# hellovuong/ORB_SLAM3_FAST

Measured on AMD Instinct MI355X. Metric: ORB extract+match frames/sec @1280×720 stereo (both-eye ORBextractor + ComputeStereoMatches), higher is better.
Workload: dtype u8; 1 GPU; C3: synthetic 1280x720 rectified stereo pairs, 1500 features, 8 levels, scale 1.2, FAST 20/7, ComputeStereoMatches (bf=0.12*532.03, b=0.12); handles=4, distinct_streams_per_gpu=32, frames_in_ring=3, stereo_matches_pair0=987, parallelism=independent stereo pairs sharded across GPUs, no data-path collective

## Files before the change

orb_slam3_fast_amd/csrc/orbx_kernels.hip:

```cpp
#include <type_traits>
#include <map>
#include <mutex>

#include "orbx_device.h"
#include "orbx_introsort.h"
#include "orbx_sincos.h"
#include "orbx_blur_mfma.h"

namespace orbx {

__constant__ int c_umax[16] = {15, 15, 15, 15, 14, 14, 14, 13, 13, 12, 11, 10, 9, 8, 6, 3};

#define RS_DW 256
#define RS_DR 16
#define RS_HROWS 6
struct ResizeLv {
  struct { int w, h, pitch, xcoef, ycoef; } D;
  struct { int w, h; } S;
  int sp, l;
  int nbx;
  const uint8_t* src; long long srcImg;
  uint8_t* dst; long long dstImg;
  const uint32_t* tiles;
  const uint32_t* rows;
// ... 683 lines not shown
  o.cpos = take(maxn * 8);
  o.e[0] = take(maxn * 8);
  o.e[1] = take(maxn * 8);
  o.mark = take(maxn * 2);
  o.bestk = take(maxn * 4);
  o.tsum = take(256 * 8 + 64);
  o.cellpre = take((maxcells + 1) * 4);
  o.total = off;
  return o;
}
__host__ __device__ inline int oct_maxn(const Geom& g, int l0, int l1) {
  int q = 0;
  for (int l = l0; l < l1; l++) q = g.lv[l].quota > q ? g.lv[l].quota : q;
  return q + 4 * kMaxIni + 8;
}
__host__ __device__ inline int oct_maxcells(const Geom& g, int l0, int l1) {
  int c = 0;
  for (int l = l0; l < l1; l++) c = g.lv[l].nCols * g.lv[l].nRows > c ? g.lv[l].nCols * g.lv[l].nRows : c;
  return c;
}
__host__ __device__ inline int oct_rep(const Geom& g, int l0, int l1) {
  const int maxn = oct_maxn(g, l0, l1), maxcells = oct_maxcells(g, l0, l1);
  if (oct_layout(maxn, maxcells, 2).total <= 78 * 1024) return 2;
  return 1;
}
size_t octree_lds_bytes(const Geom& g, int l0, int l1) {
  return (size_t)oct_layout(oct_maxn(g, l0, l1), oct_maxcells(g, l0, l1), oct_rep(g, l0, l1)).total;
}

__device__ __forceinline__ uint64_t wave0_scan_u64(uint64_t* v, int n) {
  const int lane = threadIdx.x;
  const uint64_t s = lane < n ? v[lane] : 0;
  const uint64_t incl = wave_scan_dpp_u64(s);
  if (lane < n) v[lane] = incl - s;
  return readlane_u64(incl, 63);
}
template <int NT>
__device__ __forceinline__ uint64_t block_scan_u64(uint64_t* v, int n, uint64_t* tsum) {
  const int tid = threadIdx.x, lane = tid & 63, wv = tid >> 6;
  const int per = (n + NT - 1) / NT;
  const int b = min(tid * per, n), e = min(b + per, n);
  uint64_t s = 0;
  for (int i = b; i < e; i++) s += v[i];
  const uint64_t incl = wave_scan_dpp_u64(s);
  if (lane == 63) tsum[wv] = incl;
  __syncthreads();
  uint64_t wbase = 0, total = 0;
#pragma unroll
  for (int w = 0; w < NT / 64; w++) {
    const uint64_t t = tsum[w];
    if (w < wv) wbase += t;
    total += t;
  }
  uint64_t run = wbase + incl - s;
  for (int i = b; i < e; i++) {
    const uint64_t t = v[i];
    v[i] = run;
    run += t;
  }
  __syncthreads();
  return total;
}

__device__ __forceinline__ int quadrant(int x, int y, int x0, int x1, int y0, int y1) {
  const int hx = (x1 - x0 + 1) >> 1, hy = (y1 - y0 + 1) >> 1;
  return (x < x0 + hx ? 0 : 1) | (y < y0 + hy ? 0 : 2);
}

constexpr int OCT_KMAX = 32;
constexpr int OCT_GROUP = 4;
template <bool REG, int NT>
struct OctCands {
  uint32_t rk[REG ? OCT_KMAX : 1];
  uint32_t rn2[REG ? OCT_KMAX / 2 : 1];
  uint32_t* keys;
  uint16_t* kn;
  int n;
  static constexpr uint32_t kNoCand = 0xFFFFu;
  template <class F>
  __device__ __forceinline__ void sweep(F f) {
    if constexpr (REG) {
#pragma unroll
      for (int j0 = 0; j0 < OCT_KMAX; j0 += OCT_GROUP) {
        if (j0 * NT >= n) continue;
#pragma unroll
        for (int j = j0; j < j0 + OCT_GROUP; j++)
        {
          uint32_t key = rk[j], nd = (rn2[j >> 1] >> (16 * (j & 1))) & 0xFFFFu;
          asm volatile("" : "+v"(key), "+v"(nd));
          if (nd != kNoCand) {
            f(0, key, nd);
            rn2[j >> 1] = (j & 1) ? (rn2[j >> 1] & 0xFFFFu) | (nd << 16) : (rn2[j >> 1] & 0xFFFF0000u) | nd;
          }
        }
        __builtin_amdgcn_sched_barrier(0);
      }
    } else {
      for (int k = threadIdx.x; k < n; k += NT) {
        uint32_t nd = kn[k];
        const uint32_t nd0 = nd;
        f(k, keys[k], nd);
        if (nd != nd0) kn[k] = (uint16_t)nd;
      }
    }
  }
  template <class F>
  __device__ __forceinline__ void fill(F f) {
    if constexpr (REG) {
#pragma unroll
      for (int j = 0; j < OCT_KMAX; j++) {
        const int k = (int)threadIdx.x + j * NT;
        rk[j] = 0;
        if (k < n) rk[j] = f(k);
      }
#pragma unroll
      for (int j = 0; j < OCT_KMAX; j++) {
        const int k = (int)threadIdx.x + j * NT;
        const uint32_t nd = k < n ? 0u : kNoCand;
        rn2[j >> 1] = (j & 1) ? rn2[j >> 1] | (nd << 16) : nd;
      }
    } else {
      for (int k = threadIdx.x; k < n; k += NT) {
        keys[k] = f(k);
        kn[k] = 0;
      }
    }
  }
};

struct OctCtx {
  int16_t *nx0, *nx1, *ny0, *ny1;
  uint32_t* ncnt;
  int nodeStride;
  uint32_t* cnt4;
  int nrep;
  uint32_t* cntr;
  uint16_t* cpos;
  uint64_t* scan;
  uint64_t* ebuf;
  uint16_t* mark;
  uint32_t* nmid;
  uint64_t* tsum;
  int* cellpre;
  int* s_i;
  int maxn;
  uint16_t* owner;
  int ownerBytes;
  uint8_t* tab;
  int tabBytes;
};

template <int NT, class CD>
__device__ __forceinline__ void octree_gather(CD& cd, const OctCtx& c, const LevelDev& L, int n, int cells,
                                              const uint32_t* __restrict__ sparse) {
  if (2 * n <= c.ownerBytes) {
    for (int cell = threadIdx.x; cell < cells; cell += NT) {
      const int b = c.cellpre[cell], e = min(c.cellpre[cell + 1], n);
      for (int i = b; i < e; i++) c.owner[i] = (uint16_t)cell;
    }
    __syncthreads();
    cd.fill([&](int k) {
      const int cell = c.owner[k];
      return sparse[(long long)cell * L.cellCap + (k - c.cellpre[cell])];
    });
    __syncthreads();
  } else {
    cd.fill([&](int k) {
      int lo = 0, hi = cells;
      while (hi - lo > 1) {
        const int mid = (lo + hi) >> 1;
        if (c.cellpre[mid] <= k) lo = mid; else hi = mid;
      }
      return sparse[(long long)lo * L.cellCap + (k - c.cellpre[lo])];
    });
  }
}

template <bool REG, int NT>
__device__ __forceinline__ void octree_body(const Geom& g, const LevelDev& L, const OctCtx& c, int n, int cells,
                                            const uint32_t* __restrict__ sparse, uint32_t* __restrict__ keys,
                                            uint16_t* __restrict__ kn, uint32_t* __restrict__ out,
                                            int* __restrict__ outCount, int profLevel) {
  const int tid = threadIdx.x;
#ifdef OCT_PROF
  long long tmk[96]; int nmk = 0;
#define MK() do { if (nmk < 96) tmk[nmk++] = wall_clock64(); } while (0)
#else
#define MK() do {} while (0)
#endif
  MK();
  OctCands<REG, NT> cd;
  cd.keys = keys;
  cd.kn = kn;
  cd.n = n;
  octree_gather<NT>(cd, c, L, n, cells, sparse);
  MK();
  const int N = L.quota;
  struct Buf {
    char* base;
    int stride;
    __device__ __forceinline__ int16_t* operator[](int b) const { return reinterpret_cast<int16_t*>(base + b * stride); }
  };
  struct BufU {
    char* base;
    int stride;
    __device__ __forceinline__ uint32_t* operator[](int b) const { return reinterpret_cast<uint32_t*>(base + b * stride); }
  };
  const Buf nx0{(char*)c.nx0, c.nodeStride}, nx1{(char*)c.nx1, c.nodeStride}, ny0{(char*)c.ny0, c.nodeStride},
      ny1{(char*)c.ny1, c.nodeStride};
  const BufU ncnt{(char*)c.ncnt, c.nodeStride};
  uint32_t* cnt4 = c.cnt4;
  uint32_t* cntr = c.cntr;
  const int nrep = c.nrep, rep = tid & (nrep - 1);
  auto zero_counters = [&](int nslots) {
    for (int i = tid; i < nslots * nrep; i += NT) cntr[i] = 0;
  };
  auto reduce_counters = [&](int nslots) {
    for (int i = tid; i < nslots; i += NT) {
      uint32_t v = 0;
      for (int r = 0; r < nrep; r++) v += cntr[i * nrep + r];
      cnt4[i] = v;
    }
  };
  uint16_t* cpos = c.cpos;
  uint64_t* scan = c.scan;
  uint16_t* mark = c.mark;
  uint32_t* nmid = c.nmid;
  uint64_t* tsum = c.tsum;
  auto pack_mid = [&](int b, int i) {
    const int x0 = nx0[b][i], x1 = nx1[b][i], y0 = ny0[b][i], y1 = ny1[b][i];
    return (uint32_t)(x0 + ((x1 - x0 + 1) >> 1)) | ((uint32_t)(y0 + ((y1 - y0 + 1) >> 1)) << 12) |
           (ncnt[b][i] > 1 ? 0x80000000u : 0u);
  };
  auto classify = [&](uint32_t key, uint32_t mid) {
    return (key_x(key) >= (int)(mid & 0xFFF) ? 1 : 0) | (key_y(key) >= (int)((mid >> 12) & 0xFFF) ? 2 : 0);
  };
  int* s_i = c.s_i;

  const int W = L.w - 2 * kBorder, H = L.h - 2 * kBorder;
  const int nIni = (int)roundf((float)W / (float)H);
  const float hX = (float)W / (float)nIni;

  zero_counters(kMaxIni);
  __syncthreads();
  cd.sweep([&](int, uint32_t key, uint32_t& nd) {
    const int r = (int)((float)key_x(key) / hX);
    nd = (uint32_t)r;
    atomicAdd(&cntr[r * nrep + rep], 1u);
  });
  __syncthreads();
  reduce_counters(kMaxIni);
  __syncthreads();
  if (tid == 0) {
    int na = 0;
    for (int i = 0; i < nIni; i++) {
      if (cnt4[i] == 0) {
        cpos[i] = 0xFFFF;
        continue;
      }
      nx0[0][na] = (int16_t)(int)(hX * (float)i);
      nx1[0][na] = (int16_t)(int)(hX * (float)(i + 1));
      ny0[0][na] = 0;
      ny1[0][na] = (int16_t)H;
      ncnt[0][na] = cnt4[i];
      cpos[i] = (uint16_t)na;
      na++;
    }
    s_i[0] = na;
    for (int i = 0; i < na; i++) nmid[i] = pack_mid(0, i);
  }
  __syncthreads();
  cd.sweep([&](int, uint32_t, uint32_t& nd) { nd = cpos[nd]; });
  int nA = s_i[0];
  int cur = 0;
  __syncthreads();

  MK();
  bool finish = false;
  int nE = 0, ecur = 0;
  while (!finish) {
    const int prevSize = nA;
    zero_counters(nA * 4);
    __syncthreads();
    MK();
    cd.sweep([&](int, uint32_t key, uint32_t& nd) {
      const uint32_t mid = nmid[nd];
      if (mid >> 31) {
        const int q = classify(key, mid);
        atomicAdd(&cntr[(nd * 4 + q) * nrep + rep], 1u);
        nd |= (uint32_t)q << 14;
      }
    });
    __syncthreads();
    reduce_counters(nA * 4);
    __syncthreads();
    MK();
    for (int i = tid; i < nA; i += NT) {
      uint64_t cc = 0, nm = 1, ce = 0;
      if (ncnt[cur][i] > 1) {
        nm = 0;
        for (int q = 0; q < 4; q++) {
          cc += cnt4[i * 4 + q] > 0;
          ce += cnt4[i * 4 + q] > 1;
        }
      }
      scan[i] = cc | (nm << 21) | (ce << 42);
    }
    __syncthreads();
    const uint64_t tot = block_scan_u64<NT>(scan, nA, tsum);
    MK();
    const int tc = (int)(tot & 0x1FFFFF), tnm = (int)((tot >> 21) & 0x1FFFFF), tce = (int)(tot >> 42);
    const int nxt = cur ^ 1;
    for (int i = tid; i < nA; i += NT) {
      const uint64_t pre = scan[i];
      const int pc = (int)(pre & 0x1FFFFF), pnm = (int)((pre >> 21) & 0x1FFFFF), pce = (int)(pre >> 42);
      if (ncnt[cur][i] > 1) {
        const int x0 = nx0[cur][i], x1 = nx1[cur][i], y0 = ny0[cur][i], y1 = ny1[cur][i];
        const int hx = (x1 - x0 + 1) >> 1, hy = (y1 - y0 + 1) >> 1;
        int cc = 0;
        for (int q = 0; q < 4; q++) cc += cnt4[i * 4 + q] > 0;
        const int base = tc - (pc + cc);
        int after = 0, eb = pce;
        for (int q = 0; q < 4; q++) {
          const uint32_t cq = cnt4[i * 4 + q];
          if (cq > 1) {
            int rank_after = 0;
            for (int q2 = q + 1; q2 < 4; q2++) rank_after += cnt4[i * 4 + q2] > 0;
            const int cx0 = (q & 1) ? x0 + hx : x0;
            (c.ebuf + ecur * c.maxn)[eb++] = ((uint64_t)cq << 28) | ((uint64_t)(uint32_t)cx0 << 16) | (uint64_t)(base + rank_after);
          }
        }
        for (int q = 3; q >= 0; q--) {
          const uint32_t cq = cnt4[i * 4 + q];
          if (cq == 0) continue;
          const int pos = base + after++;
          nx0[nxt][pos] = (int16_t)((q & 1) ? x0 + hx : x0);
          nx1[nxt][pos] = (int16_t)((q & 1) ? x1 : x0 + hx);
          ny0[nxt][pos] = (int16_t)((q & 2) ? y0 + hy : y0);
          ny1[nxt][pos] = (int16_t)((q & 2) ? y1 : y0 + hy);
          ncnt[nxt][pos] = cq;
          cpos[i * 4 + q] = (uint16_t)pos;
        }
      } else {
        const int pos = tc + pnm;
        nx0[nxt][pos] = nx0[cur][i];
        nx1[nxt][pos] = nx1[cur][i];
        ny0[nxt][pos] = ny0[cur][i];
        ny1[nxt][pos] = ny1[cur][i];
// ... 54 lines not shown
    __syncthreads();
    for (int m = tid; m < nE; m += NT) {
      const int nd = (int)(E[nE - 1 - m] & 0xFFFF);
      uint64_t cc = 0, ce = 0;
      for (int q = 0; q < 4; q++) {
        cc += cnt4[nd * 4 + q] > 0;
        ce += cnt4[nd * 4 + q] > 1;
      }
      scan[m] = cc | (ce << 21);
    }
    __syncthreads();
    block_scan_u64<NT>(scan, nE, tsum);
    for (int m = tid; m < nE; m += NT) {
      const int nd = (int)(E[nE - 1 - m] & 0xFFFF);
      int cc = 0;
      for (int q = 0; q < 4; q++) cc += cnt4[nd * 4 + q] > 0;
      const int cincl = (int)(scan[m] & 0x1FFFFF) + cc;
      if (nA + cincl - (m + 1) >= N) {
        atomicMin(&s_i[1], m + 1);
        s_i[2] = 1;
      }
    }
    __syncthreads();
    const int nP = s_i[1];
    const bool broke = s_i[2] != 0;
    int tc, tce;
    if (nP < nE) {
      tc = (int)(scan[nP] & 0x1FFFFF);
      tce = (int)(scan[nP] >> 21);
    } else {
      const int nd = (int)(E[0] & 0xFFFF);
      int cc = 0, ce = 0;
      for (int q = 0; q < 4; q++) {
        cc += cnt4[nd * 4 + q] > 0;
        ce += cnt4[nd * 4 + q] > 1;
      }
      tc = nE ? (int)(scan[nE - 1] & 0x1FFFFF) + cc : 0;
      tce = nE ? (int)(scan[nE - 1] >> 21) + ce : 0;
    }
    const int nxt = cur ^ 1;
    for (int m = tid; m < nP; m += NT) {
      const int nd = (int)(E[nE - 1 - m] & 0xFFFF);
      const int x0 = nx0[cur][nd], x1 = nx1[cur][nd], y0 = ny0[cur][nd], y1 = ny1[cur][nd];
      const int hx = (x1 - x0 + 1) >> 1, hy = (y1 - y0 + 1) >> 1;
      int cc = 0;
      for (int q = 0; q < 4; q++) cc += cnt4[nd * 4 + q] > 0;
      const int pc = (int)(scan[m] & 0x1FFFFF);
      int eb = (int)(scan[m] >> 21);
      const int base = tc - (pc + cc);
      for (int q = 0; q < 4; q++) {
        const uint32_t cq = cnt4[nd * 4 + q];
        if (cq > 1) {
          int rank_after = 0;
          for (int q2 = q + 1; q2 < 4; q2++) rank_after += cnt4[nd * 4 + q2] > 0;
          const int cx0 = (q & 1) ? x0 + hx : x0;
          E2[eb++] = ((uint64_t)cq << 28) | ((uint64_t)(uint32_t)cx0 << 16) | (uint64_t)(base + rank_after);
        }
      }
      int after = 0;
      for (int q = 3; q >= 0; q--) {
        const uint32_t cq = cnt4[nd * 4 + q];
        if (cq == 0) continue;
        const int pos = base + after++;
        nx0[nxt][pos] = (int16_t)((q & 1) ? x0 + hx : x0);
        nx1[nxt][pos] = (int16_t)((q & 1) ? x1 : x0 + hx);
        ny0[nxt][pos] = (int16_t)((q & 2) ? y0 + hy : y0);
        ny1[nxt][pos] = (int16_t)((q & 2) ? y1 : y0 + hy);
        ncnt[nxt][pos] = cq;
        cpos[nd * 4 + q] = (uint16_t)pos;
      }
    }
    __syncthreads();
    for (int i = tid; i < nA; i += NT) scan[i] = (mark[i] == 0 || mark[i] > nP) ? 1 : 0;
    __syncthreads();
    const int nKeep = (int)block_scan_u64<NT>(scan, nA, tsum);
    for (int i = tid; i < nA; i += NT) {
      if (mark[i] == 0 || mark[i] > nP) {
        const int pos = tc + (int)scan[i];
        nx0[nxt][pos] = nx0[cur][i];
        nx1[nxt][pos] = nx1[cur][i];
        ny0[nxt][pos] = ny0[cur][i];
        ny1[nxt][pos] = ny1[cur][i];
        ncnt[nxt][pos] = ncnt[cur][i];
        cpos[i * 4] = cpos[i * 4 + 1] = cpos[i * 4 + 2] = cpos[i * 4 + 3] = (uint16_t)pos;
      }
    }
    __syncthreads();
    cd.sweep([&](int, uint32_t, uint32_t& v) { v = cpos[(v & 0x3FFF) * 4 + (v >> 14)]; });
    for (int i = tid; i < tc + nKeep; i += NT) nmid[i] = pack_mid(nxt, i);
    __syncthreads();
    cur = nxt;
    nA = tc + nKeep;
    nE = tce;
    ecur ^= 1;
    MK();
    if (broke || nA == prevSize) finish = true;
  }

  MK();
  uint64_t* best = scan;
  uint64_t* bestr = reinterpret_cast<uint64_t*>(cntr);
  const int nrepB = nrep >= 2 ? nrep * 2 : 1, repB = tid & (nrepB - 1);
  if (nrepB > 1)
    for (int i = tid; i < nA * nrepB; i += NT) bestr[i] = 0;
  else
    for (int i = tid; i < nA; i += NT) best[i] = 0;
  __syncthreads();
  const float invH = 1.0f / (float)L.hCell, invW = 1.0f / (float)L.wCell;
  auto rank_key = [&](uint32_t key) {
    const int xr = key_x(key) - 3, yr = key_y(key) - 3;
    const int cy = (int)(((float)yr + 0.5f) * invH), cx = (int)(((float)xr + 0.5f) * invW);
    const uint32_t rank = (uint32_t)(((cy * L.nCols + cx) * L.hCell + (yr - cy * L.hCell)) * L.wCell + (xr - cx * L.wCell));
    return ((unsigned long long)key_r(key) << 32) | (0xFFFFFFFFu - rank);
  };
  if (nrepB > 1) {
    cd.sweep([&](int, uint32_t key, uint32_t& nd) {
      atomicMax((unsigned long long*)&bestr[nd * nrepB + repB], rank_key(key));
    });
    __syncthreads();
    for (int i = tid; i < nA; i += NT) {
      uint64_t v = 0;
      for (int r = 0; r < nrepB; r++) v = bestr[i * nrepB + r] > v ? bestr[i * nrepB + r] : v;
      best[i] = v;
    }
  } else {
    cd.sweep([&](int, uint32_t key, uint32_t& nd) { atomicMax((unsigned long long*)&best[nd], rank_key(key)); });
  }
  __syncthreads();
  const int nOut = min(nA, L.selCap);
  cd.sweep([&](int, uint32_t key, uint32_t& nd) {
    if ((int)nd < nOut && best[nd] == rank_key(key)) out[nd] = pack_key(key_x(key) + kBorder, key_y(key) + kBorder, key_r(key));
  });
  if (tid == 0) *outCount = nOut;
  MK();
#ifdef OCT_PROF
  if (tid == 0 && profLevel) {
    printf("n=%d nA=%d :", n, nA);
    for (int i = 1; i < nmk; i++) printf(" %d", (int)(tmk[i] - tmk[i - 1]));
    printf("\n");
  }
#endif
#undef MK
}

constexpr int OCT_HD = 5;
__host__ __device__ inline int oct_hbase(int nIni, int d) { return nIni * (((1 << (2 * d)) - 1) / 3); }
__host__ __device__ inline bool oct_hist_fits(int nIni) {
  return nIni <= 2 && oct_hbase(nIni, OCT_HD + 1) * 6 <= 16400 && nIni * (1 << (2 * OCT_HD)) * 2 <= 4096;
}

template <int NT>
__device__ __forceinline__ bool octree_hist_body(const Geom& g, const LevelDev& L, const OctCtx& c, int n, int cells,
                                                 const uint32_t* __restrict__ sparse, uint32_t* __restrict__ keys,
                                                 uint32_t* __restrict__ out, int* __restrict__ outCount, int prof) {
  const int tid = threadIdx.x;
#ifdef OCT_PROF
  long long hmk[48]; int nhmk = 0;
#define HMK() do { if (nhmk < 48) hmk[nhmk++] = wall_clock64(); } while (0)
#else
#define HMK() do {} while (0)
#endif
  HMK();
  OctCands<true, NT> cd;
  cd.keys = keys;
  cd.kn = nullptr;
  cd.n = n;
  octree_gather<NT>(cd, c, L, n, cells, sparse);
  HMK();
  const int N = L.quota;
  struct Buf {
    char* base;
    int stride;
    __device__ __forceinline__ int16_t* operator[](int b) const { return reinterpret_cast<int16_t*>(base + b * stride); }
  };
  struct BufU {
    char* base;
    int stride;
    __device__ __forceinline__ uint32_t* operator[](int b) const { return reinterpret_cast<uint32_t*>(base + b * stride); }
  };
  const Buf nx0{(char*)c.nx0, c.nodeStride}, nx1{(char*)c.nx1, c.nodeStride}, ny0{(char*)c.ny0, c.nodeStride},
      ny1{(char*)c.ny1, c.nodeStride};
  const BufU ncnt{(char*)c.ncnt, c.nodeStride};
  const int W = L.w - 2 * kBorder, H = L.h - 2 * kBorder;
  const int nIni = (int)roundf((float)W / (float)H);
  const float hX = (float)W / (float)nIni;
  uint32_t* hist = c.cntr;
  uint16_t* leafAt = reinterpret_cast<uint16_t*>(hist + oct_hbase(nIni, OCT_HD + 1));
  uint16_t* t5 = reinterpret_cast<uint16_t*>(c.cnt4);
  uint16_t* ndcBuf = c.cpos;
  auto ndc = [&](int b) { return ndcBuf + b * c.maxn; };
  uint64_t* scan = c.scan;
  uint16_t* mark = c.mark;
  uint64_t* tsum = c.tsum;
  int* s_i = c.s_i;
  const int nH = oct_hbase(nIni, OCT_HD + 1);
  for (int i = tid; i < nH; i += NT) hist[i] = 0;
  if (tid == 0) s_i[3] = 0;
  const bool pathTab = 2 * (W + H) + 8 <= c.tabBytes;
  uint16_t* px = reinterpret_cast<uint16_t*>(c.tab);
  uint16_t* py = px + ((W + 3) & ~3);
  auto x_path = [&](int x) {
    const int r = (int)((float)x / hX);
    int x0 = (int)(hX * (float)r), x1 = (int)(hX * (float)(r + 1));
    uint32_t code = (uint32_t)r;
#pragma unroll
    for (int d = 0; d < OCT_HD; d++) {
      const int mx = x0 + ((x1 - x0 + 1) >> 1);
      const int qx = x >= mx;
      x0 = qx ? mx : x0;
      x1 = qx ? x1 : mx;
      code = code * 4 + (uint32_t)qx;
    }
    return code;
  };
  auto y_path = [&](int y) {
    int y0 = 0, y1 = H;
    uint32_t code = 0;
#pragma unroll
    for (int d = 0; d < OCT_HD; d++) {
      const int my = y0 + ((y1 - y0 + 1) >> 1);
      const int qy = y >= my;
      y0 = qy ? my : y0;
      y1 = qy ? y1 : my;
      code = code * 4 + (uint32_t)(qy << 1);
    }
    return code;
  };
  if (pathTab) {
    for (int i = tid; i < W + H; i += NT) {
      if (i < W) px[i] = (uint16_t)x_path(i);
      else py[i - W] = (uint16_t)y_path(i - W);
    }
  }
  __syncthreads();
  {
    uint32_t* h5 = hist + oct_hbase(nIni, OCT_HD);
    if (pathTab) {
      cd.sweep([&](int, uint32_t key, uint32_t& nd) {
        const uint32_t code = (uint32_t)px[key_x(key)] + (uint32_t)py[key_y(key)];
        nd = code;
        atomicAdd(&h5[code], 1u);
      });
    } else {
      cd.sweep([&](int, uint32_t key, uint32_t& nd) {
        const uint32_t code = x_path(key_x(key)) + y_path(key_y(key));
        nd = code;
        atomicAdd(&h5[code], 1u);
      });
    }
  }
  __syncthreads();
  HMK();
  for (int d = OCT_HD - 1; d >= 0; d--) {
    const uint32_t* ch = hist + oct_hbase(nIni, d + 1);
    uint32_t* pa = hist + oct_hbase(nIni, d);
    for (int i = tid; i < (nIni << (2 * d)); i += NT) pa[i] = ch[4 * i] + ch[4 * i + 1] + ch[4 * i + 2] + ch[4 * i + 3];
    __syncthreads();
  }
  auto child_count = [&](uint32_t dc, int q) {
    const int d = (int)(dc >> 13);
    return hist[oct_hbase(nIni, d + 1) + (int)(dc & 0x1FFF) * 4 + q];
  };
  if (tid == 0) {
    int na = 0;
    for (int i = 0; i < nIni; i++) {
      if (hist[i] == 0) continue;
      nx0[0][na] = (int16_t)(int)(hX * (float)i);
      nx1[0][na] = (int16_t)(int)(hX * (float)(i + 1));
      ny0[0][na] = 0;
      ny1[0][na] = (int16_t)H;
      ncnt[0][na] = hist[i];
      ndc(0)[na] = (uint16_t)i;
      na++;
    }
    s_i[0] = na;
  }
  __syncthreads();
  int nA = s_i[0];
  int cur = 0;
  bool finish = false;
  int nE = 0, ecur = 0;
  HMK();
  auto pass = [&](auto waveTag) -> int {
    constexpr bool kWave = decltype(waveTag)::value;
    auto sync = [&]() {
      if (kWave) {
        __builtin_amdgcn_fence(__ATOMIC_ACQ_REL, "workgroup");
        __builtin_amdgcn_wave_barrier();
      } else {
        __syncthreads();
      }
    };
    const int prevSize = nA;
      for (int i = tid; i < nA; i += NT) {
        uint64_t cc = 0, nm = 1, ce = 0;
        if (ncnt[cur][i] > 1) {
          nm = 0;
          const uint32_t dc = ndc(cur)[i];
          if ((dc >> 13) >= (uint32_t)OCT_HD) {
            s_i[3] = 1;
          } else {
            for (int q = 0; q < 4; q++) {
              const uint32_t cq = child_count(dc, q);
              cc += cq > 0;
              ce += cq > 1;
            }
          }
        }
        scan[i] = cc | (nm << 21) | (ce << 42);
      }
      sync();
      if (s_i[3]) return 3;
      const uint64_t tot = kWave ? wave0_scan_u64(scan, nA) : block_scan_u64<NT>(scan, nA, tsum);
      const int tc = (int)(tot & 0x1FFFFF), tnm = (int)((tot >> 21) & 0x1FFFFF), tce = (int)(tot >> 42);
      const int nxt = cur ^ 1;
      for (int i = tid; i < nA; i += NT) {
        const uint64_t pre = scan[i];
        const int pc = (int)(pre & 0x1FFFFF), pnm = (int)((pre >> 21) & 0x1FFFFF), pce = (int)(pre >> 42);
        if (ncnt[cur][i] > 1) {
          const uint32_t dc = ndc(cur)[i];
          const uint32_t cdc = (((dc >> 13) + 1) << 13) | ((dc & 0x1FFF) * 4);
          const int x0 = nx0[cur][i], x1 = nx1[cur][i], y0 = ny0[cur][i], y1 = ny1[cur][i];
          const int hx = (x1 - x0 + 1) >> 1, hy = (y1 - y0 + 1) >> 1;
          uint32_t cq4[4];
          int cc = 0;
          for (int q = 0; q < 4; q++) {
            cq4[q] = child_count(dc, q);
            cc += cq4[q] > 0;
          }
          const int base = tc - (pc + cc);
          int after = 0, eb = pce;
          for (int q = 0; q < 4; q++) {
            if (cq4[q] > 1) {
              int rank_after = 0;
              for (int q2 = q + 1; q2 < 4; q2++) rank_after += cq4[q2] > 0;
              const int cx0 = (q & 1) ? x0 + hx : x0;
              (c.ebuf + ecur * c.maxn)[eb++] = ((uint64_t)cq4[q] << 28) | ((uint64_t)(uint32_t)cx0 << 16) | (uint64_t)(base + rank_after);
            }
          }
          for (int q = 3; q >= 0; q--) {
            if (cq4[q] == 0) continue;
            const int pos = base + after++;
            nx0[nxt][pos] = (int16_t)((q & 1) ? x0 + hx : x0);
            nx1[nxt][pos] = (int16_t)((q & 1) ? x1 : x0 + hx);
            ny0[nxt][pos] = (int16_t)((q & 2) ? y0 + hy : y0);
            ny1[nxt][pos] = (int16_t)((q & 2) ? y1 : y0 + hy);
            ncnt[nxt][pos] = cq4[q];
            ndc(nxt)[pos] = (uint16_t)(cdc + q);
          }
        } else {
          const int pos = tc + pnm;
          nx0[nxt][pos] = nx0[cur][i];
          nx1[nxt][pos] = nx1[cur][i];
          ny0[nxt][pos] = ny0[cur][i];
          ny1[nxt][pos] = ny1[cur][i];
          ncnt[nxt][pos] = ncnt[cur][i];
          ndc(nxt)[pos] = ndc(cur)[i];
        }
      }
    sync();
    cur = nxt;
    nA = tc + tnm;
    nE = tce;
    if (nA >= N || nA == prevSize) return 1;
    if (nA + 3 * nE > N) return 2;
    return 0;
  };
  int state = 0;
  if (nA <= 64) {
    if (tid < 64) {
      while (state == 0 && nA <= 64) state = pass(std::true_type{});
      if (tid == 0) {
        s_i[4] = state;
        s_i[5] = nA;
        s_i[6] = nE;
        s_i[7] = cur;
      }
    }
    __syncthreads();
    state = s_i[4];
    nA = s_i[5];
    nE = s_i[6];
    cur = s_i[7];
  }
  while (state == 0) state = pass(std::false_type{});
  if (state == 3) return false;
  finish = state == 1;
  HMK();
  while (!finish) {
    const int prevSize = nA;
    uint64_t* E = c.ebuf + ecur * c.maxn;
    uint64_t* E2 = c.ebuf + (ecur ^ 1) * c.maxn;
    introsort_block(E, nE, E2, reinterpret_cast<uint16_t*>(scan), reinterpret_cast<uint16_t*>(scan) + c.maxn + 4,
                    reinterpret_cast<uint32_t*>(tsum), NT);
    HMK();
    if (tid == 0) {
      s_i[1] = nE;
      s_i[2] = 0;
    }
    for (int i = tid; i < nA; i += NT) mark[i] = 0;
    __syncthreads();
    for (int m = tid; m < nE; m += NT) {
      const int nd = (int)(E[nE - 1 - m] & 0xFFFF);
      mark[nd] = (uint16_t)(m + 1);
      const uint32_t dc = ndc(cur)[nd];
      uint64_t cc = 0, ce = 0;
      if ((dc >> 13) >= (uint32_t)OCT_HD) {
        s_i[3] = 1;
      } else {
        for (int q = 0; q < 4; q++) {
          const uint32_t cq = child_count(dc, q);
          cc += cq > 0;
          ce += cq > 1;
        }
      }
      scan[m] = cc | (ce << 21);
    }
    __syncthreads();
    if (s_i[3]) return false;
    block_scan_u64<NT>(scan, nE, tsum);
    for (int m = tid; m < nE; m += NT) {
      const int nd = (int)(E[nE - 1 - m] & 0xFFFF);
      const uint32_t dc = ndc(cur)[nd];
      int cc = 0;
      for (int q = 0; q < 4; q++) cc += child_count(dc, q) > 0;
      const int cincl = (int)(scan[m] & 0x1FFFFF) + cc;
      if (nA + cincl - (m + 1) >= N) {
        atomicMin(&s_i[1], m + 1);
        s_i[2] = 1;
      }
    }
    __syncthreads();
    const int nP = s_i[1];
    const bool broke = s_i[2] != 0;
    int tc, tce;
    if (nP < nE) {
      tc = (int)(scan[nP] & 0x1FFFFF);
      tce = (int)(scan[nP] >> 21);
    } else {
      int cc = 0, ce = 0;
      if (nE) {
        const uint32_t dc = ndc(cur)[(int)(E[0] & 0xFFFF)];
        for (int q = 0; q < 4; q++) {
          const uint32_t cq = child_count(dc, q);
          cc += cq > 0;
          ce += cq > 1;
        }
      }
      tc = nE ? (int)(scan[nE - 1] & 0x1FFFFF) + cc : 0;
      tce = nE ? (int)(scan[nE - 1] >> 21) + ce : 0;
    }
    const int nxt = cur ^ 1;
    for (int m = tid; m < nP; m += NT) {
      const int nd = (int)(E[nE - 1 - m] & 0xFFFF);
      const uint32_t dc = ndc(cur)[nd];
      const uint32_t cdc = (((dc >> 13) + 1) << 13) | ((dc & 0x1FFF) * 4);
      const int x0 = nx0[cur][nd], x1 = nx1[cur][nd], y0 = ny0[cur][nd], y1 = ny1[cur][nd];
      const int hx = (x1 - x0 + 1) >> 1, hy = (y1 - y0 + 1) >> 1;
      uint32_t cq4[4];
      int cc = 0;
      for (int q = 0; q < 4; q++) {
        cq4[q] = child_count(dc, q);
        cc += cq4[q] > 0;
      }
      const int pc = (int)(scan[m] & 0x1FFFFF);
      int eb = (int)(scan[m] >> 21);
      const int base = tc - (pc + cc);
      for (int q = 0; q < 4; q++) {
        if (cq4[q] > 1) {
          int rank_after = 0;
          for (int q2 = q + 1; q2 < 4; q2++) rank_after += cq4[q2] > 0;
          const int cx0 = (q & 1) ? x0 + hx : x0;
          E2[eb++] = ((uint64_t)cq4[q] << 28) | ((uint64_t)(uint32_t)cx0 << 16) | (uint64_t)(base + rank_after);
        }
      }
      int after = 0;
      for (int q = 3; q >= 0; q--) {
        if (cq4[q] == 0) continue;
        const int pos = base + after++;
        nx0[nxt][pos] = (int16_t)((q & 1) ? x0 + hx : x0);
        nx1[nxt][pos] = (int16_t)((q & 1) ? x1 : x0 + hx);
        ny0[nxt][pos] = (int16_t)((q & 2) ? y0 + hy : y0);
        ny1[nxt][pos] = (int16_t)((q & 2) ? y1 : y0 + hy);
        ncnt[nxt][pos] = cq4[q];
        ndc(nxt)[pos] = (uint16_t)(cdc + q);
      }
    }
    __syncthreads();
    for (int i = tid; i < nA; i += NT) scan[i] = (mark[i] == 0 || mark[i] > nP) ? 1 : 0;
    __syncthreads();
    const int nKeep = (int)block_scan_u64<NT>(scan, nA, tsum);
    for (int i = tid; i < nA; i += NT) {
      if (mark[i] == 0 || mark[i] > nP) {
        const int pos = tc + (int)scan[i];
        nx0[nxt][pos] = nx0[cur][i];
        nx1[nxt][pos] = nx1[cur][i];
        ny0[nxt][pos] = ny0[cur][i];
        ny1[nxt][pos] = ny1[cur][i];
        ncnt[nxt][pos] = ncnt[cur][i];
        ndc(nxt)[pos] = ndc(cur)[i];
      }
    }
    __syncthreads();
    cur = nxt;
    nA = tc + nKeep;
    nE = tce;
    ecur ^= 1;
    if (broke || nA == prevSize) finish = true;
    HMK();
  }
  for (int i = tid; i < nH; i += NT) leafAt[i] = 0xFFFF;
  __syncthreads();
  for (int i = tid; i < nA; i += NT) {
    const uint32_t dc = ndc(cur)[i];
    leafAt[oct_hbase(nIni, (int)(dc >> 13)) + (int)(dc & 0x1FFF)] = (uint16_t)i;
  }
  __syncthreads();
  for (int c5 = tid; c5 < (nIni << (2 * OCT_HD)); c5 += NT) {
    uint16_t v = 0xFFFF;
#pragma unroll
    for (int d = OCT_HD; d >= 0; d--) {
      const uint16_t w = leafAt[oct_hbase(nIni, d) + (c5 >> (2 * (OCT_HD - d)))];
      v = v == 0xFFFF ? w : v;
    }
    t5[c5] = v;
  }
  __syncthreads();
  HMK();
  uint64_t* best = scan;
  uint64_t* bestr = reinterpret_cast<uint64_t*>(c.cntr);
  const int nrepB = c.nrep >= 2 ? c.nrep * 2 : 1, repB = tid & (nrepB - 1);
  if (nrepB > 1)
    for (int i = tid; i < nA * nrepB; i += NT) bestr[i] = 0;
  else
    for (int i = tid; i < nA; i += NT) best[i] = 0;
  __syncthreads();
  const float invH = 1.0f / (float)L.hCell, invW = 1.0f / (float)L.wCell;
  auto rank_key = [&](uint32_t key) {
    const int xr = key_x(key) - 3, yr = key_y(key) - 3;
    const int cy = (int)(((float)yr + 0.5f) * invH), cx = (int)(((float)xr + 0.5f) * invW);
    const uint32_t rank = (uint32_t)(((cy * L.nCols + cx) * L.hCell + (yr - cy * L.hCell)) * L.wCell + (xr - cx * L.wCell));
    return ((unsigned long long)key_r(key) << 32) | (0xFFFFFFFFu - rank);
  };
  cd.sweep([&](int, uint32_t key, uint32_t& nd) {
    const uint32_t fn = t5[nd];
    if (nrepB > 1) atomicMax((unsigned long long*)&bestr[fn * nrepB + repB], rank_key(key));
    else atomicMax((unsigned long long*)&best[fn], rank_key(key));
  });
  __syncthreads();
  const int nOut = min(nA, L.selCap);
  for (int i = tid; i < nOut; i += NT) {
    uint64_t v = nrepB > 1 ? 0 : best[i];
    if (nrepB > 1)
      for (int r = 0; r < nrepB; r++) v = bestr[i * nrepB + r] > v ? bestr[i * nrepB + r] : v;
    const uint32_t rank = 0xFFFFFFFFu - (uint32_t)v, resp = (uint32_t)(v >> 32);
    const uint32_t xloc = rank % (uint32_t)L.wCell, t1 = rank / (uint32_t)L.wCell;
    const uint32_t yloc = t1 % (uint32_t)L.hCell, t2 = t1 / (uint32_t)L.hCell;
    const uint32_t cx = t2 % (uint32_t)L.nCols, cy = t2 / (uint32_t)L.nCols;
    out[i] = pack_key((int)(cx * L.wCell + xloc) + 3 + kBorder, (int)(cy * L.hCell + yloc) + 3 + kBorder, (int)resp);
  }
  if (tid == 0) *outCount = nOut;
  HMK();
#ifdef OCT_PROF
  if (tid == 0 && prof) {
    printf("hist n=%d nA=%d :", n, nA);
    for (int i = 1; i < nhmk; i++) printf(" %d", (int)(hmk[i] - hmk[i - 1]));
    printf("  (x10 ns: gather | sweep1 | sums+roots | phase 1 | {sort, rest} per phase-2 round | leaf table | best sweeps)\n");
  }
#endif
#undef HMK
  return true;
}

template <int NT>
__device__ __forceinline__ void octree_block(const Geom& g, const uint32_t* __restrict__ cellCand,
                                             const int* __restrict__ cellCount, uint32_t* __restrict__ cand,
                                             int* __restrict__ candCount, uint16_t* __restrict__ knode,
                                             uint32_t* __restrict__ sel, int* __restrict__ selCount, int profLevel,
                                             int forceGlobal, int level0, int nlv, uint8_t* smem, int* s_i) {
  const int tid = threadIdx.x;
#ifdef OCT_WG_PROF
  struct WgPrint {
    long long t0;
    int l, img, on;
    __device__ ~WgPrint() {
      if (on) printf("octwg level %d img %d start %lld end %lld\n", l, img, t0 % 100000000, wall_clock64() % 100000000);
    }
  } wgPrint{wall_clock64(), 0, 0, (int)(threadIdx.x == 0)};
#endif
  const int nimg_ = gridDim.x / nlv;
  const int l = level0 + blockIdx.x / nimg_, img = blockIdx.x % nimg_;
#ifdef OCT_WG_PROF
  wgPrint.l = l;
  wgPrint.img = img;
#endif
  const LevelDev L = g.lv[l];
  const int maxn = oct_maxn(g, level0, level0 + nlv);
  const int nrep = oct_rep(g, level0, level0 + nlv);
  const OctLds o = oct_layout(maxn, oct_maxcells(g, level0, level0 + nlv), nrep);
  OctCtx c;
  c.nx0 = (int16_t*)(smem + o.nx0[0]);
  c.nx1 = (int16_t*)(smem + o.nx1[0]);
  c.ny0 = (int16_t*)(smem + o.ny0[0]);
  c.ny1 = (int16_t*)(smem + o.ny1[0]);
  c.ncnt = (uint32_t*)(smem + o.ncnt[0]);
  c.nodeStride = o.nx0[1] - o.nx0[0];
  c.ebuf = (uint64_t*)(smem + o.e[0]);
  c.cnt4 = (uint32_t*)(smem + o.cnt4);
  c.cntr = (uint32_t*)(smem + o.cntr);
  c.nrep = nrep;
  c.cpos = (uint16_t*)(smem + o.cpos);
  c.scan = (uint64_t*)(smem + o.scan);
  c.mark = (uint16_t*)(smem + o.mark);
  c.nmid = (uint32_t*)(smem + o.bestk);
  c.tsum = (uint64_t*)(smem + o.tsum);
  c.cellpre = (int*)(smem + o.cellpre);
  c.s_i = s_i;
  c.maxn = maxn;
  c.owner = (uint16_t*)smem;
  c.ownerBytes = o.tsum;
  c.tab = smem + o.cpos;
  c.tabBytes = o.tsum - o.cpos;

  const int cells = L.nCols * L.nRows;
  int n;
  {
    const int* cc = cellCount + (long long)img * g.totalCells + L.cellStart;
    const int per = (cells + NT - 1) / NT;
    const int cb = min(tid * per, cells), ce = min(cb + per, cells);
    int sum = 0;
    for (int ci = cb; ci < ce; ci++) sum += cc[ci];
    const int incl = wave_scan_dpp(sum);
    if ((tid & 63) == 63) c.tsum[tid >> 6] = (uint64_t)incl;
    __syncthreads();
    int wbase = 0, total = 0;
#pragma unroll
    for (int w = 0; w < NT / 64; w++) {
      const int t = (int)c.tsum[w];
      if (w < (tid >> 6)) wbase += t;
      total += t;
    }
    n = min(total, L.candCap);
    int run = wbase + incl - sum;
    for (int ci = cb; ci < ce; ci++) {
      c.cellpre[ci] = run;
      run += cc[ci];
    }
    if (tid == 0) {
      c.cellpre[cells] = total;
      candCount[img * g.nlevels + l] = n;
    }
    __syncthreads();
  }
  const uint32_t* sparse = cellCand + (long long)img * g.cellImg + L.cellOff;
  uint32_t* keys = cand + (long long)img * g.candImg + L.candOff;
  uint16_t* kn = knode + (long long)img * g.candImg + L.candOff;
  uint32_t* out = sel + (long long)img * g.selImg + L.selOff;
  int* outCount = selCount + img * g.nlevels + l;
  if (n <= OCT_KMAX * NT && forceGlobal != 1) {
    const int W = L.w - 2 * kBorder, H = L.h - 2 * kBorder;
    const int nIni = (int)roundf((float)W / (float)H);
    bool done = false;
    if (forceGlobal == 0 && oct_hist_fits(nIni)) {
      done = octree_hist_body<NT>(g, L, c, n, cells, sparse, keys, out, outCount, profLevel == l && img == 0);
      __syncthreads();
    }
    if (!done) octree_body<true, NT>(g, L, c, n, cells, sparse, keys, kn, out, outCount, profLevel == l && img == 0);
  } else {
    octree_body<false, NT>(g, L, c, n, cells, sparse, keys, kn, out, outCount, profLevel == l && img == 0);
  }
}

template <int NT>
__global__ __launch_bounds__(NT, 4) void k_octree(Geom g, const uint32_t* __restrict__ cellCand,
                                                const int* __restrict__ cellCount, int* __restrict__ cellPrefix,
                                                uint32_t* __restrict__ cand, int* __restrict__ candCount,
                                                uint16_t* __restrict__ knode, uint32_t* __restrict__ sel,
                                                int* __restrict__ selCount, int profLevel, int forceGlobal, int level0,
                                                int nlv) {
  extern __shared__ __attribute__((aligned(16))) uint8_t smem[];
  __shared__ int s_i[8];
  octree_block<NT>(g, cellCand, cellCount, cand, candCount, knode, sel, selCount, profLevel, forceGlobal, level0, nlv, smem, s_i);
}

__global__ __launch_bounds__(512, 4) void k_octree_mixed(Geom g, const uint32_t* __restrict__ cellCand,
                                                         const int* __restrict__ cellCount, uint32_t* __restrict__ cand,
                                                         int* __restrict__ candCount, uint16_t* __restrict__ knode,
                                                         uint32_t* __restrict__ sel, int* __restrict__ selCount,
                                                         int profLevel, int forceGlobal, uint32_t classes) {
  extern __shared__ __attribute__((aligned(16))) uint8_t smem[];
  __shared__ int s_i[8];
  const int l = blockIdx.x / (gridDim.x / g.nlevels);
  const int nt = 128 << ((classes >> (2 * l)) & 3u);
  if ((int)threadIdx.x >= nt) return;
  if (nt == 512)
    octree_block<512>(g, cellCand, cellCount, cand, candCount, knode, sel, selCount, profLevel, forceGlobal, 0, g.nlevels, smem, s_i);
  else if (nt == 256)
    octree_block<256>(g, cellCand, cellCount, cand, candCount, knode, sel, selCount, profLevel, forceGlobal, 0, g.nlevels, smem, s_i);
  else
    octree_block<128>(g, cellCand, cellCount, cand, candCount, knode, sel, selCount, profLevel, forceGlobal, 0, g.nlevels, smem, s_i);
}

static int g_octree_force_global_host = 0;
void debug_set_octree_global(int on) { g_octree_force_global_host = on < 0 ? 0 : (on > 2 ? 2 : on); }
static int g_octree_class_host = 0;
void debug_set_octree_class(int nt) { g_octree_class_host = (nt == 128 || nt == 256 || nt == 512) ? nt : 0; }
int debug_octree_class() { return g_octree_class_host; }

constexpr int kOctArea256 = 300000, kOctArea128 = 70000;
void build_octree_plan(const Geom& g, OctPlan& p) {
  int prev = 512;
  for (int l = 0; l < g.nlevels; l++) {
    const long long area = (long long)(g.lv[l].w - 2 * kBorder) * (g.lv[l].h - 2 * kBorder);
    const int nt = area > kOctArea256 ? 512 : (area > kOctArea128 ? 256 : 128);
    prev = p.nt[l] = nt < prev ? nt : prev;
    p.lds[l] = (int)octree_lds_bytes(g, 0, g.nlevels);
  }
}

template <int NT>
static hipError_t launch_octree_nt(const Geom& g, int nimg, const uint32_t* cellCand, const int* cellCount, int* cellPrefix,
                                   uint32_t* cand, int* candCount, uint16_t* knode, uint32_t* sel, int* selCount, int level0,
                                   int level1, hipStream_t s) {
  dim3 grid((level1 - level0) * nimg);
#ifdef OCT_PROF
  static const int profLevel = getenv("ORBX_OCTREE_PROF_LEVEL") ? atoi(getenv("ORBX_OCTREE_PROF_LEVEL")) : 0;
#else
  const int profLevel = -1;
#endif
  const size_t lds = octree_lds_bytes(g, level0, level1);
  if (g_octree_class_host) {
    const hipError_t e = raise_dynamic_lds(reinterpret_cast<const void*>(k_octree<NT>), lds);
    if (e != hipSuccess) return e;
  }
  hipLaunchKernelGGL(k_octree<NT>, grid, dim3(NT), lds, s, g, cellCand, cellCount, cellPrefix, cand, candCount, knode, sel,
                     selCount, profLevel, g_octree_force_global_host, level0, level1 - level0);
  return hipGetLastError();
}
hipError_t launch_octree_mixed(const Geom& g, const OctPlan& plan, int nimg, const uint32_t* cellCand, const int* cellCount,
                               uint32_t* cand, int* candCount, uint16_t* knode, uint32_t* sel, int* selCount, hipStream_t s) {
  uint32_t classes = 0;
  for (int l = 0; l < g.nlevels; l++) classes |= (plan.nt[l] == 512 ? 2u : (plan.nt[l] == 256 ? 1u : 0u)) << (2 * l);
#ifdef OCT_PROF
  static const int profLevel = getenv("ORBX_OCTREE_PROF_LEVEL") ? atoi(getenv("ORBX_OCTREE_PROF_LEVEL")) : 0;
#else
  const int profLevel = -1;
#endif
  hipLaunchKernelGGL(k_octree_mixed, dim3(g.nlevels * nimg), dim3(512), octree_lds_bytes(g, 0, g.nlevels), s, g, cellCand,
                     cellCount, cand, candCount, knode, sel, selCount, profLevel, g_octree_force_global_host, classes);
  return hipGetLastError();
}
hipError_t launch_octree(const Geom& g, int nimg, const uint32_t* cellCand, const int* cellCount, int* cellPrefix,
                         uint32_t* cand, int* candCount, uint16_t* knode, uint32_t* sel, int* selCount, int level0,
                         int level1, int nt, hipStream_t s) {
  if (level1 <= level0) return hipSuccess;
  if (nt == 128)
    return launch_octree_nt<128>(g, nimg, cellCand, cellCount, cellPrefix, cand, candCount, knode, sel, selCount, level0, level1, s);
  if (nt == 256)
    return launch_octree_nt<256>(g, nimg, cellCand, cellCount, cellPrefix, cand, candCount, knode, sel, selCount, level0, level1, s);
  if (nt == 512)
    return launch_octree_nt<512>(g, nimg, cellCand, cellCount, cellPrefix, cand, candCount, knode, sel, selCount, level0, level1, s);
  return hipErrorInvalidValue;
}

__device__ __forceinline__ int reflect101(int p, int n) {
  if (p < 0) p = -p;
  if (p >= n) p = 2 * n - 2 - p;
  return p;
}

#define BL_TW 128
#define BL_TH 32
template <bool T440>
__global__ __launch_bounds__(256) void k_blur(Geom g, Pyr p, int level0, int level1, int xcdRun) {
  constexpr uint32_t kT2 = T440 ? 49u : 48u, kT3 = T440 ? 55u : 56u;
  __shared__ uint32_t in[BL_TH + 6][BL_TW / 4 + 2 + 1];
  __shared__ uint32_t hp[(BL_TH + 6) / 2][BL_TW + 1];
  const int tid = threadIdx.x;
  const int img = blockIdx.z;
  int tile = xcd_run_remap_rt(blockIdx.x, gridDim.x, blockIdx.z, xcdRun);
  int l = level0;
  for (;; l++) {
    const int tx = (g.lv[l].w + BL_TW - 1) / BL_TW, ty = (g.lv[l].h + BL_TH - 1) / BL_TH;
    if (tile < tx * ty || l + 1 == level1) break;
    tile -= tx * ty;
  }
  const LevelDev L = g.lv[l];
  const int tx = (L.w + BL_TW - 1) / BL_TW;
  if (tile >= tx * ((L.h + BL_TH - 1) / BL_TH)) return;
  const int x0 = (tile % tx) * BL_TW, y0 = (tile / tx) * BL_TH;
  const int bodyEnd = T440 && g.cv440 > 1 ? (L.w & ~(g.cv440 - 1)) : 0;
  int pitch;
  const uint8_t* im = level_ptr(g, p, img, l, pitch);
  constexpr int IW = BL_TW / 4 + 2;
  if (x0 >= 4 && y0 >= 3 && x0 + BL_TW + 4 <= L.w && y0 + BL_TH + 3 <= L.h) {
    const int c = tid % IW, r0 = tid / IW;
    if (r0 < 7) {
      const uint8_t* src = im + (long long)(y0 - 3 + r0) * pitch + (x0 - 4) + 4 * c;
#pragma unroll
      for (int k = 0; k < 6; k++) {
        const int r = r0 + 7 * k;
        if (r < BL_TH + 6) in[r][c] = *reinterpret_cast<const uint32_t*>(src + (long long)(7 * k) * pitch);
      }
    }
  } else {
    for (int i = tid; i < (BL_TH + 6) * IW; i += 256) {
      const int r = i / IW, c = i - r * IW;
      const int y = y0 + r - 3, x = x0 - 4 + 4 * c;
      uint32_t v;
      if (y >= 0 && y < L.h && x >= 0 && x + 4 <= L.w) {
        v = *reinterpret_cast<const uint32_t*>(im + (long long)y * pitch + x);
      } else {
        const int yy = reflect101(min(max(y, -3), L.h + 2), L.h);
        v = 0;
#pragma unroll
        for (int k = 0; k < 4; k++) {
          const int xx = reflect101(min(max(x + k, -3), L.w + 2), L.w);
          v |= (uint32_t)im[(long long)yy * pitch + xx] << (8 * k);
        }
      }
      in[r][c] = v;
    }
// ... 637 lines not shown
```

Baseline: 84620 stereo frames/s.

## Trim barriers and redundant passes in octree distribution kernel

Fuses the candidate-owner fill into the cell prefix-count loop, keeping per-thread cell counts in registers so the gather skips a separate pass and barrier. In the wave-wide split pass, each thread keeps its first node's counts in registers and uses a DPP wave scan with a ballot instead of an LDS scan and barrier. It also moves the leafAt init and mark reset earlier so they share existing barriers, and uses a separate keep buffer so one sync can be dropped. The main risk is hazards from the removed barriers (shared-memory aliasing of owner, cnt4 and keep) and extra register pressure.

```diff
diff --git a/orb_slam3_fast_amd/csrc/orbx_kernels.hip b/orb_slam3_fast_amd/csrc/orbx_kernels.hip
--- a/orb_slam3_fast_amd/csrc/orbx_kernels.hip
+++ b/orb_slam3_fast_amd/csrc/orbx_kernels.hip
@@ -859,13 +859,15 @@
 
 template <int NT, class CD>
 __device__ __forceinline__ void octree_gather(CD& cd, const OctCtx& c, const LevelDev& L, int n, int cells,
-                                              const uint32_t* __restrict__ sparse) {
+                                              const uint32_t* __restrict__ sparse, bool ownerDone) {
   if (2 * n <= c.ownerBytes) {
-    for (int cell = threadIdx.x; cell < cells; cell += NT) {
-      const int b = c.cellpre[cell], e = min(c.cellpre[cell + 1], n);
-      for (int i = b; i < e; i++) c.owner[i] = (uint16_t)cell;
-    }
-    __syncthreads();
+    if (!ownerDone) {
+      for (int cell = threadIdx.x; cell < cells; cell += NT) {
+        const int b = c.cellpre[cell], e = min(c.cellpre[cell + 1], n);
+        for (int i = b; i < e; i++) c.owner[i] = (uint16_t)cell;
+      }
+      __syncthreads();
+    }
     cd.fill([&](int k) {
       const int cell = c.owner[k];
       return sparse[(long long)cell * L.cellCap + (k - c.cellpre[cell])];
@@ -887,7 +889,7 @@
 __device__ __forceinline__ void octree_body(const Geom& g, const LevelDev& L, const OctCtx& c, int n, int cells,
                                             const uint32_t* __restrict__ sparse, uint32_t* __restrict__ keys,
                                             uint16_t* __restrict__ kn, uint32_t* __restrict__ out,
-                                            int* __restrict__ outCount, int profLevel) {
+                                            int* __restrict__ outCount, int profLevel, bool ownerDone) {
   const int tid = threadIdx.x;
 #ifdef OCT_PROF
   long long tmk[96]; int nmk = 0;
@@ -900,7 +902,7 @@
   cd.keys = keys;
   cd.kn = kn;
   cd.n = n;
-  octree_gather<NT>(cd, c, L, n, cells, sparse);
+  octree_gather<NT>(cd, c, L, n, cells, sparse, ownerDone);
   MK();
   const int N = L.quota;
   struct Buf {
@@ -1261,7 +1263,8 @@
 template <int NT>
 __device__ __forceinline__ bool octree_hist_body(const Geom& g, const LevelDev& L, const OctCtx& c, int n, int cells,
                                                  const uint32_t* __restrict__ sparse, uint32_t* __restrict__ keys,
-                                                 uint32_t* __restrict__ out, int* __restrict__ outCount, int prof) {
+                                                 uint32_t* __restrict__ out, int* __restrict__ outCount, int prof,
+                                                 bool ownerDone) {
   const int tid = threadIdx.x;
 #ifdef OCT_PROF
   long long hmk[48]; int nhmk = 0;
@@ -1274,7 +1277,7 @@
   cd.keys = keys;
   cd.kn = nullptr;
   cd.n = n;
-  octree_gather<NT>(cd, c, L, n, cells, sparse);
+  octree_gather<NT>(cd, c, L, n, cells, sparse, ownerDone);
   HMK();
   const int N = L.quota;
   struct Buf {
@@ -1303,7 +1306,10 @@
   uint64_t* tsum = c.tsum;
   int* s_i = c.s_i;
   const int nH = oct_hbase(nIni, OCT_HD + 1);
-  for (int i = tid; i < nH; i += NT) hist[i] = 0;
+  for (int i = tid; i < nH; i += NT) {
+    hist[i] = 0;
+    leafAt[i] = 0xFFFF;
+  }
   if (tid == 0) s_i[3] = 0;
   const bool pathTab = 2 * (W + H) + 8 <= c.tabBytes;
   uint16_t* px = reinterpret_cast<uint16_t*>(c.tab);
@@ -1401,72 +1407,103 @@
       }
     };
     const int prevSize = nA;
-      for (int i = tid; i < nA; i += NT) {
-        uint64_t cc = 0, nm = 1, ce = 0;
-        if (ncnt[cur][i] > 1) {
-          nm = 0;
-          const uint32_t dc = ndc(cur)[i];
-          if ((dc >> 13) >= (uint32_t)OCT_HD) {
-            s_i[3] = 1;
-          } else {
-            for (int q = 0; q < 4; q++) {
-              const uint32_t cq = child_count(dc, q);
-              cc += cq > 0;
-              ce += cq > 1;
-            }
-          }
-        }
-        scan[i] = cc | (nm << 21) | (ce << 42);
-      }
-      sync();
-      if (s_i[3]) return 3;
-      const uint64_t tot = kWave ? wave0_scan_u64(scan, nA) : block_scan_u64<NT>(scan, nA, tsum);
-      const int tc = (int)(tot & 0x1FFFFF), tnm = (int)((tot >> 21) & 0x1FFFFF), tce = (int)(tot >> 42);
-      const int nxt = cur ^ 1;
-      for (int i = tid; i < nA; i += NT) {
-        const uint64_t pre = scan[i];
-        const int pc = (int)(pre & 0x1FFFFF), pnm = (int)((pre >> 21) & 0x1FFFFF), pce = (int)(pre >> 42);
-        if (ncnt[cur][i] > 1) {
-          const uint32_t dc = ndc(cur)[i];
-          const uint32_t cdc = (((dc >> 13) + 1) << 13) | ((dc & 0x1FFF) * 4);
-          const int x0 = nx0[cur][i], x1 = nx1[cur][i], y0 = ny0[cur][i], y1 = ny1[cur][i];
-          const int hx = (x1 - x0 + 1) >> 1, hy = (y1 - y0 + 1) >> 1;
-          uint32_t cq4[4];
-          int cc = 0;
+    uint32_t fCnt = 0, fDc = 0, fq0 = 0, fq1 = 0, fq2 = 0, fq3 = 0;
+    uint64_t fPk = 0;
+    bool deep = false;
+    for (int i = tid; i < nA; i += NT) {
+      uint64_t cc = 0, nm = 1, ce = 0;
+      const uint32_t cn = ncnt[cur][i];
+      uint32_t dc = 0, cq4[4] = {0, 0, 0, 0};
+      if (cn > 1) {
+        nm = 0;
+        dc = ndc(cur)[i];
+        if ((dc >> 13) >= (uint32_t)OCT_HD) {
+          s_i[3] = 1;
+          deep = true;
+        } else {
           for (int q = 0; q < 4; q++) {
             cq4[q] = child_count(dc, q);
             cc += cq4[q] > 0;
+            ce += cq4[q] > 1;
           }
-          const int base = tc - (pc + cc);
-          int after = 0, eb = pce;
-          for (int q = 0; q < 4; q++) {
-            if (cq4[q] > 1) {
-              int rank_after = 0;
-              for (int q2 = q + 1; q2 < 4; q2++) rank_after += cq4[q2] > 0;
-              const int cx0 = (q & 1) ? x0 + hx : x0;
-              (c.ebuf + ecur * c.maxn)[eb++] = ((uint64_t)cq4[q] << 28) | ((uint64_t)(uint32_t)cx0 << 16) | (uint64_t)(base + rank_after);
-            }
+        }
+      }
+      const uint64_t pk = cc | (nm << 21) | (ce << 42);
+      if (i == tid) {
+        fCnt = cn;
+        fDc = dc;
+        fq0 = cq4[0];
+        fq1 = cq4[1];
+        fq2 = cq4[2];
+        fq3 = cq4[3];
+        fPk = pk;
+      }
+      if (!kWave) scan[i] = pk;
+    }
+    uint64_t tot, fPre = 0;
+    if (kWave) {
+      if (__ballot(deep)) return 3;
+      const uint64_t incl = wave_scan_dpp_u64(fPk);
+      fPre = incl - fPk;
+      tot = readlane_u64(incl, 63);
+    } else {
+      sync();
+      if (s_i[3]) return 3;
+      tot = block_scan_u64<NT>(scan, nA, tsum);
+    }
+    const int tc = (int)(tot & 0x1FFFFF), tnm = (int)((tot >> 21) & 0x1FFFFF), tce = (int)(tot >> 42);
+    const int nxt = cur ^ 1;
+    for (int i = tid; i < nA; i += NT) {
+      const bool first = i == tid;
+      const uint64_t pre = kWave ? fPre : scan[i];
+      const int pc = (int)(pre & 0x1FFFFF), pnm = (int)((pre >> 21) & 0x1FFFFF), pce = (int)(pre >> 42);
+      const uint32_t cn = first ? fCnt : ncnt[cur][i];
+      if (cn > 1) {
+        const uint32_t dc = first ? fDc : ndc(cur)[i];
+        const uint32_t cdc = (((dc >> 13) + 1) << 13) | ((dc & 0x1FFF) * 4);
+        const int x0 = nx0[cur][i], x1 = nx1[cur][i], y0 = ny0[cur][i], y1 = ny1[cur][i];
+        const int hx = (x1 - x0 + 1) >> 1, hy = (y1 - y0 + 1) >> 1;
+        uint32_t cq4[4];
+        if (first) {
+          cq4[0] = fq0;
+          cq4[1] = fq1;
+          cq4[2] = fq2;
+          cq4[3] = fq3;
+        } else {
+          for (int q = 0; q < 4; q++) cq4[q] = child_count(dc, q);
+        }
+        int cc = 0;
+        for (int q = 0; q < 4; q++) cc += cq4[q] > 0;
+        const int base = tc - (pc + cc);
+        int after = 0, eb = pce;
+        for (int q = 0; q < 4; q++) {
+          if (cq4[q] > 1) {
+            int rank_after = 0;
+            for (int q2 = q + 1; q2 < 4; q2++) rank_after += cq4[q2] > 0;
+            const int cx0 = (q & 1) ? x0 + hx : x0;
+            (c.ebuf + ecur * c.maxn)[eb++] = ((uint64_t)cq4[q] << 28) | ((uint64_t)(uint32_t)cx0 << 16) | (uint64_t)(base + rank_after);
           }
-          for (int q = 3; q >= 0; q--) {
-            if (cq4[q] == 0) continue;
-            const int pos = base + after++;
-            nx0[nxt][pos] = (int16_t)((q & 1) ? x0 + hx : x0);
-            nx1[nxt][pos] = (int16_t)((q & 1) ? x1 : x0 + hx);
-            ny0[nxt][pos] = (int16_t)((q & 2) ? y0 + hy : y0);
-            ny1[nxt][pos] = (int16_t)((q & 2) ? y1 : y0 + hy);
-            ncnt[nxt][pos] = cq4[q];
-            ndc(nxt)[pos] = (uint16_t)(cdc + q);
-          }
-        } else {
-          const int pos = tc + pnm;
-          nx0[nxt][pos] = nx0[cur][i];
-          nx1[nxt][pos] = nx1[cur][i];
-          ny0[nxt][pos] = ny0[cur][i];
-          ny1[nxt][pos] = ny1[cur][i];
-          ncnt[nxt][pos] = ncnt[cur][i];
-          ndc(nxt)[pos] = ndc(cur)[i];
         }
-      }
+        for (int q = 3; q >= 0; q--) {
+          if (cq4[q] == 0) continue;
+          const int pos = base + after++;
+          nx0[nxt][pos] = (int16_t)((q & 1) ? x0 + hx : x0);
+          nx1[nxt][pos] = (int16_t)((q & 1) ? x1 : x0 + hx);
+          ny0[nxt][pos] = (int16_t)((q & 2) ? y0 + hy : y0);
+          ny1[nxt][pos] = (int16_t)((q & 2) ? y1 : y0 + hy);
+          ncnt[nxt][pos] = cq4[q];
+          ndc(nxt)[pos] = (uint16_t)(cdc + q);
+        }
+      } else {
+        const int pos = tc + pnm;
+        nx0[nxt][pos] = nx0[cur][i];
+        nx1[nxt][pos] = nx1[cur][i];
+        ny0[nxt][pos] = ny0[cur][i];
+        ny1[nxt][pos] = ny1[cur][i];
+        ncnt[nxt][pos] = cn;
+        ndc(nxt)[pos] = ndc(cur)[i];
+      }
+    }
     sync();
     cur = nxt;
     nA = tc + tnm;
@@ -1500,15 +1537,14 @@
     const int prevSize = nA;
     uint64_t* E = c.ebuf + ecur * c.maxn;
     uint64_t* E2 = c.ebuf + (ecur ^ 1) * c.maxn;
+    if (tid == 0) {
+      s_i[1] = nE;
+      s_i[2] = 0;
+    }
+    for (int i = tid; i < nA; i += NT) mark[i] = 0;
     introsort_block(E, nE, E2, reinterpret_cast<uint16_t*>(scan), reinterpret_cast<uint16_t*>(scan) + c.maxn + 4,
                     reinterpret_cast<uint32_t*>(tsum), NT);
     HMK();
-    if (tid == 0) {
-      s_i[1] = nE;
-      s_i[2] = 0;
-    }
-    for (int i = tid; i < nA; i += NT) mark[i] = 0;
-    __syncthreads();
     for (int m = tid; m < nE; m += NT) {
       const int nd = (int)(E[nE - 1 - m] & 0xFFFF);
       mark[nd] = (uint16_t)(m + 1);
@@ -1595,13 +1631,13 @@
         ndc(nxt)[pos] = (uint16_t)(cdc + q);
       }
     }
+    uint64_t* keep = reinterpret_cast<uint64_t*>(c.cnt4);
+    for (int i = tid; i < nA; i += NT) keep[i] = (mark[i] == 0 || mark[i] > nP) ? 1 : 0;
     __syncthreads();
-    for (int i = tid; i < nA; i += NT) scan[i] = (mark[i] == 0 || mark[i] > nP) ? 1 : 0;
-    __syncthreads();
-    const int nKeep = (int)block_scan_u64<NT>(scan, nA, tsum);
+    const int nKeep = (int)block_scan_u64<NT>(keep, nA, tsum);
     for (int i = tid; i < nA; i += NT) {
       if (mark[i] == 0 || mark[i] > nP) {
-        const int pos = tc + (int)scan[i];
+        const int pos = tc + (int)keep[i];
         nx0[nxt][pos] = nx0[cur][i];
         nx1[nxt][pos] = nx1[cur][i];
         ny0[nxt][pos] = ny0[cur][i];
@@ -1618,8 +1654,6 @@
     if (broke || nA == prevSize) finish = true;
     HMK();
   }
-  for (int i = tid; i < nH; i += NT) leafAt[i] = 0xFFFF;
-  __syncthreads();
   for (int i = tid; i < nA; i += NT) {
     const uint32_t dc = ndc(cur)[i];
     leafAt[oct_hbase(nIni, (int)(dc >> 13)) + (int)(dc & 0x1FFF)] = (uint16_t)i;
@@ -1733,27 +1767,55 @@
 
   const int cells = L.nCols * L.nRows;
   int n;
+  bool ownerDone = false;
   {
     const int* cc = cellCount + (long long)img * g.totalCells + L.cellStart;
     const int per = (cells + NT - 1) / NT;
     const int cb = min(tid * per, cells), ce = min(cb + per, cells);
+    constexpr int kPerReg = 4;
+    const bool inReg = per <= kPerReg;
+    int cnt[kPerReg];
     int sum = 0;
-    for (int ci = cb; ci < ce; ci++) sum += cc[ci];
+    if (inReg) {
+#pragma unroll
+      for (int j = 0; j < kPerReg; j++) {
+        cnt[j] = cb + j < ce ? cc[cb + j] : 0;
+        sum += cnt[j];
+      }
+    } else {
+      for (int ci = cb; ci < ce; ci++) sum += cc[ci];
+    }
     const int incl = wave_scan_dpp(sum);
-    if ((tid & 63) == 63) c.tsum[tid >> 6] = (uint64_t)incl;
+    int* wsum = reinterpret_cast<int*>(c.tsum);
+    if ((tid & 63) == 63) wsum[tid >> 6] = incl;
     __syncthreads();
     int wbase = 0, total = 0;
 #pragma unroll
     for (int w = 0; w < NT / 64; w++) {
-      const int t = (int)c.tsum[w];
+      const int t = wsum[w];
       if (w < (tid >> 6)) wbase += t;
       total += t;
     }
     n = min(total, L.candCap);
     int run = wbase + incl - sum;
-    for (int ci = cb; ci < ce; ci++) {
-      c.cellpre[ci] = run;
-      run += cc[ci];
+    if (inReg) {
+      ownerDone = 2 * n <= c.ownerBytes;
+#pragma unroll
+      for (int j = 0; j < kPerReg; j++) {
+        if (cb + j < ce) {
+          c.cellpre[cb + j] = run;
+          if (ownerDone) {
+            const int e = min(run + cnt[j], n);
+            for (int i = run; i < e; i++) c.owner[i] = (uint16_t)(cb + j);
+          }
+          run += cnt[j];
+        }
+      }
+    } else {
+      for (int ci = cb; ci < ce; ci++) {
+        c.cellpre[ci] = run;
+        run += cc[ci];
+      }
     }
     if (tid == 0) {
       c.cellpre[cells] = total;
@@ -1771,12 +1833,13 @@
     const int nIni = (int)roundf((float)W / (float)H);
     bool done = false;
     if (forceGlobal == 0 && oct_hist_fits(nIni)) {
-      done = octree_hist_body<NT>(g, L, c, n, cells, sparse, keys, out, outCount, profLevel == l && img == 0);
+      done = octree_hist_body<NT>(g, L, c, n, cells, sparse, keys, out, outCount, profLevel == l && img == 0, ownerDone);
       __syncthreads();
-    }
-    if (!done) octree_body<true, NT>(g, L, c, n, cells, sparse, keys, kn, out, outCount, profLevel == l && img == 0);
+      if (!done) ownerDone = false;
+    }
+    if (!done) octree_body<true, NT>(g, L, c, n, cells, sparse, keys, kn, out, outCount, profLevel == l && img == 0, ownerDone);
   } else {
-    octree_body<false, NT>(g, L, c, n, cells, sparse, keys, kn, out, outCount, profLevel == l && img == 0);
+    octree_body<false, NT>(g, L, c, n, cells, sparse, keys, kn, out, outCount, profLevel == l && img == 0, ownerDone);
   }
 }
 
```

Measured after the change: 84610 stereo frames/s, median of 2. No clear change (-0.0%).
